# MIC-DKFZ/MultiTalent

Hardware: AMD Instinct MI355X
Metric: CT patches/s (48x192x192) train fwd+bwd (higher is better)
Workload: dtype f32; 1 GPU; Task009_Spleen Generic_UNet nc=2 softmax Dice+CE; batch_per_gpu=2, global_batch=2, parallelism=dp1, step=fwd+loss+bwd+clip12+SGD-nesterov, precision=fp32

## Files before the change

### include/mtseg.h

```cpp
#ifndef MTSEG_H
#define MTSEG_H

#include <stddef.h>
#include <stdint.h>

#ifdef __cplusplus
extern "C" {
#endif

#define MT_OK 0
#define MT_EINVAL (-1)
#define MT_EWORKSPACE (-2)
#define MT_EHIP (-3)
#define MT_EUNSUPPORTED (-4)

#define MT_ABI_VERSION 4
#define MT_MAX_CHUNKS 64

#define MT_F32 0
#define MT_BF16 1
#define MT_F16 2

typedef void* mt_stream_t;

// ... 104 lines not shown
  float* stats_part;
  int32_t odtype;
  int32_t scatter;
  int32_t mma;
} mt_pointwise_t;
int mt_pointwise_fwd(const mt_pointwise_t* p, mt_stream_t stream);
int mt_pointwise_stats_blocks(const mt_pointwise_t* p);
int mt_pointwise_io_supported(const mt_pointwise_t* p);
int mt_pointwise_pack_layout(const mt_pointwise_t* p);
int mt_head_bwd_supported(int Cin, int Cout);
size_t mt_head_bwd_workspace(int N, long V, int Cin, int Cout);
int mt_head_bwd(const mt_src_t* x, const float* dy, int dycs, int N, long V, int Cin, int Cout, const float* wpack_bwd,
                float* dx, int dxcs, int dxdtype , int accumulate_dx, float* dw,
                long s_ci, long s_co, float* dbias, int accumulate_dw, int* dbias_done, void* ws, size_t ws_bytes, mt_stream_t stream);
int mt_head_bwd_io_supported(int xdtype, int xcs, int dxdtype, int dxcs, int Cin, int Cout);


int mt_inorm_finalize(const float* part, int N, int nsb, int C, double count, const float* gamma,
                      const float* beta, float eps, float* mean, float* rstd, float* scale, float* shift,
                      mt_stream_t stream);
int mt_inorm_lrelu_apply(const float* y, int ycs, const float* scale, const float* shift, float slope,
                         const float* res, int rcs, const float* rscale, const float* rshift, float rslope,
                         float* out, int ocs, int N, long V, int C, int dtype , mt_stream_t stream);
size_t mt_inorm_bwd_workspace(int N, long V, int C);
int mt_inorm_lrelu_bwd(float* g, int gcs, const float* y, int ycs, const float* mean, const float* rstd,
                       const float* gamma, const float* beta, float slope, int N, long V, int C,
                       float* dgamma, float* dbeta, float* dbias, const float* part, int part_nblk, int part_cs, int part_c0,
                       void* ws, size_t ws_bytes, int gdtype, int ydtype , mt_stream_t stream);
int mt_lrelu_bwd(float* g, int gcs, const float* y, int ycs, const float* scale, const float* shift,
                 float slope, const float* y2, int y2cs, const float* scale2, const float* shift2,
// ... 131 lines not shown
```

### multitalent_amd/_lib.py

```python
import ctypes as C
import os

_HERE = os.path.dirname(os.path.abspath(__file__))
LIB_PATH = os.path.join(_HERE, os.environ.get('MT_LIB_VARIANT', 'libmtseg_hip.so'))

MT_MAX_CHUNKS = 64
c_float_p = C.POINTER(C.c_float)


class mt_src_t(C.Structure):
    _fields_ = [('ptr', C.c_void_p), ('cs', C.c_int32), ('C', C.c_int32), ('scale', C.c_void_p),
                ('shift', C.c_void_p), ('slope', C.c_float), ('dtype', C.c_int32)]


class mt_bwd_stats_t(C.Structure):
    _fields_ = [('y', C.c_void_p), ('mean', C.c_void_p), ('rstd', C.c_void_p), ('gamma', C.c_void_p), ('beta', C.c_void_p),
                ('ycs', C.c_int32), ('c0', C.c_int32), ('C', C.c_int32), ('slope', C.c_float)]


class mt_conv3d_t(C.Structure):
    _fields_ = [('src', mt_src_t * 2), ('nsrc', C.c_int32),
                ('N', C.c_int32), ('Di', C.c_int32), ('Hi', C.c_int32), ('Wi', C.c_int32),
                ('dilD', C.c_int32), ('dilH', C.c_int32), ('dilW', C.c_int32),
                ('Do', C.c_int32), ('Ho', C.c_int32), ('Wo', C.c_int32),
# ... 53 lines not shown
    'mt_gaussian_blur_axis': (_i, [_vp, _vp, _i, _i, _i, _i, _i, _vp, _vp]),
    'mt_conv3d_pack_layout': (_i, [_P(mt_conv3d_t)]),
    'mt_conv3d_bwd_data_strided_pack_layout': (_i, [_P(mt_conv3d_t)]),
    'mt_conv3d_kernel_name': (_i, [_P(mt_conv3d_t), C.c_char_p, _sz]),
    'mt_conv3d_bwd_stats_supported': (_i, [_P(mt_conv3d_t)]),
    'mt_conv3d_bwd_weight_kernel_name': (_i, [_P(mt_conv3d_t), _P(mt_src_t), C.c_char_p, _sz]),
    'mt_conv3d_bwd_data_strided_kernel_name': (_i, [_P(mt_conv3d_t), C.c_char_p, _sz]),
    'mt_conv3d_bwd_weight_workspace': (_sz, [_P(mt_conv3d_t)]),
    'mt_conv3d_bwd_weight': (_i, [_P(mt_conv3d_t), _P(mt_src_t), _vp, _l, _l, _l, _l, _l, _i, _vp, _sz, _vp]),
    'mt_pointwise_fwd': (_i, [_P(mt_pointwise_t), _vp]),
    'mt_pointwise_stats_blocks': (_i, [_P(mt_pointwise_t)]),
    'mt_head_bwd_supported': (_i, [_i, _i]),
    'mt_head_bwd_workspace': (_sz, [_i, _l, _i, _i]),
    'mt_head_bwd': (_i, [_P(mt_src_t), _vp, _i, _i, _l, _i, _i, _vp, _vp, _i, _i, _i, _vp, _l, _l, _vp, _i, _P(C.c_int), _vp, _sz, _vp]),
    'mt_head_bwd_io_supported': (_i, [_i, _i, _i, _i, _i, _i]),
    'mt_pointwise_io_supported': (_i, [_P(mt_pointwise_t)]),
    'mt_pointwise_pack_layout': (_i, [_P(mt_pointwise_t)]),
    'mt_inorm_finalize': (_i, [_vp, _i, _i, _i, _d, _vp, _vp, _f, _vp, _vp, _vp, _vp, _vp]),
    'mt_inorm_lrelu_apply': (_i, [_vp, _i, _vp, _vp, _f, _vp, _i, _vp, _vp, _f, _vp, _i, _i, _l, _i, _i, _vp]),
    'mt_inorm_bwd_workspace': (_sz, [_i, _l, _i]),
    'mt_inorm_lrelu_bwd': (_i, [_vp, _i, _vp, _i, _vp, _vp, _vp, _vp, _f, _i, _l, _i, _vp, _vp, _vp, _vp, _i, _i, _i, _vp, _sz, _i, _i, _vp]),
    'mt_lrelu_bwd': (_i, [_vp, _i, _vp, _i, _vp, _vp, _f, _vp, _i, _vp, _vp, _f, _vp, _i, _i, _l, _i, _i, _i, _vp]),
    'mt_lrelu_bwd_stats_blocks': (_i, [_l, _i]),
    'mt_lrelu_bwd_stats': (_i, [_vp, _vp, _vp, _vp, _f, _vp, _vp, _vp, _f, _vp, _vp, _vp, _vp, _i, _l, _i, _i, _i, _vp]),
    'mt_channel_sum_workspace': (_sz, [_i, _l, _i]),
    'mt_channel_sum': (_i, [_vp, _i, _i, _l, _i, _vp, _i, _vp, _sz, _i, _vp]),
    'mt_cast': (_i, [_vp, _i, _i, _vp, _i, _i, _l, _i, _i, _vp]),
    'mt_conv3d_io_supported': (_i, [_P(mt_conv3d_t)]),
    'mt_conv3d_bwd_data_strided_io_supported': (_i, [_P(mt_conv3d_t)]),
    'mt_conv3d_bwd_weight_io_supported': (_i, [_P(mt_conv3d_t), _P(mt_src_t)]),
# ... 105 lines not shown
```

### multitalent_amd/csrc/mt_common.h

```cpp
#pragma once
#include <hip/hip_runtime.h>
#include <stdint.h>
#include <stdio.h>
#include "../../include/mtseg.h"

typedef __attribute__((ext_vector_type(16))) float f32x16;
typedef __attribute__((ext_vector_type(4))) float f32x4;

#define MT_WAVE 64

void mt_set_error(const char* fmt, ...);

#define MT_REQUIRE(cond, ...)            \
  do {                                   \
    if (!(cond)) {                       \
      mt_set_error(__VA_ARGS__);         \
      return MT_EINVAL;                  \
    }                                    \
  } while (0)

#define MT_REQUIRE_WORKSPACE(who, have, need)                                              \
  do {                                                                                   \
    const size_t have_ = (have), need_ = (need);                                         \
    if (have_ < need_) {                                                                 \
      mt_set_error("%s: workspace of %zu bytes, %zu needed", who, have_, need_);         \
      return MT_EWORKSPACE;                                                              \
// ... 130 lines not shown
```

### multitalent_amd/csrc/norm.hip

```cpp
#include "mt_common.h"
#include <initializer_list>

__global__ __launch_bounds__(256) void inorm_finalize_kernel(const float* __restrict__ part, int nsb, int C, double count,
                                                             const float* __restrict__ gamma, const float* __restrict__ beta,
                                                             float eps, float* mean, float* rstd, float* scale, float* shift) {
  __shared__ double red[4][2];
  const int n = blockIdx.x / C, c = blockIdx.x % C;
  const float2* p = (const float2*)part + (size_t)n * nsb * C + c;
  double s1 = 0.0, s2 = 0.0;
  for (int s = threadIdx.x; s < nsb; s += 256) {
    const float2 v = p[(size_t)s * C];
    s1 += (double)v.x; s2 += (double)v.y;
  }
  s1 = mt_wave_sum_d(s1);
  s2 = mt_wave_sum_d(s2);
  if ((threadIdx.x & 63) == 0) { red[threadIdx.x >> 6][0] = s1; red[threadIdx.x >> 6][1] = s2; }
  __syncthreads();
  if (threadIdx.x == 0) {
    s1 = (red[0][0] + red[1][0]) + (red[2][0] + red[3][0]);
    s2 = (red[0][1] + red[1][1]) + (red[2][1] + red[3][1]);
    const double m = s1 / count;
    double var = s2 / count - m * m;
    if (var < 0.0) var = 0.0;
    const double rs = 1.0 / sqrt(var + (double)eps);
// ... 212 lines not shown
  a = mt_wave_sum_d(a);
  if (threadIdx.x == 0) out[c] = accumulate ? out[c] + (float)a : (float)a;
}


#define NF_UNROLL 4

struct InBwdFast {
  void* g; const void* y;
  const float* mean; const float* rstd; const float* gamma; const float* beta; float slope;
  long nvec;
  int C, G, A, nblk;
  float* part1;
  const float* m;
  float* part2;
};

template <int VEC, bool APPLY, int AT, int GT>
__global__ __launch_bounds__(256) void inorm_bwd_fast_kernel(const InBwdFast P) {
  static_assert(mt_ebytes<AT>() == mt_ebytes<GT>(), "one vector index addresses both tensors");
  __shared__ float red[256 * VEC * 2];
  const int n = blockIdx.y, t = threadIdx.x;
  const bool act = t < P.A;
  const int grp = t % P.G;
  float mu[VEC], rs[VEC], ga[VEC], be[VEC], m1[VEC], m2[VEC], a0[VEC], a1[VEC];
#pragma unroll
  for (int e = 0; e < VEC; ++e) {
    const int c = grp * VEC + e;
    mu[e] = P.mean[(size_t)n * P.C + c]; rs[e] = P.rstd[(size_t)n * P.C + c];
    ga[e] = P.gamma ? P.gamma[c] : 1.f; be[e] = P.beta ? P.beta[c] : 0.f;
    if (APPLY) { m1[e] = P.m[((size_t)n * P.C + c) * 2]; m2[e] = P.m[((size_t)n * P.C + c) * 2 + 1]; }
    a0[e] = 0.f; a1[e] = 0.f;
  }
  const long per = ((P.nvec + P.nblk - 1) / P.nblk + P.A - 1) / P.A * P.A;
  const long lo = (long)blockIdx.x * per;
  long hi = lo + per; if (hi > P.nvec) hi = P.nvec;
  const size_t sbytes = (size_t)n * P.nvec * VEC * mt_ebytes<GT>();
  char* gp = (char*)P.g + sbytes;
  const char* yp = (const char*)P.y + sbytes;
  if (act) {
    for (long i0 = lo + t; i0 < hi; i0 += (long)P.A * NF_UNROLL) {
      float gv[NF_UNROLL][VEC], yv[NF_UNROLL][VEC];
#pragma unroll
      for (int u = 0; u < NF_UNROLL; ++u) {
        const long i = i0 + (long)u * P.A;
        if (i < hi) { mt_ldv<VEC, GT>(gp, (size_t)i, gv[u]); mt_ldv<VEC, AT>(yp, (size_t)i, yv[u]); }
      }
#pragma unroll
      for (int u = 0; u < NF_UNROLL; ++u) {
        const long i = i0 + (long)u * P.A;
        if (i < hi) {
          float out[VEC];
#pragma unroll
          for (int e = 0; e < VEC; ++e) {
            const float zh = (yv[u][e] - mu[e]) * rs[e];
            const float z = fmaf(zh, ga[e], be[e]);
            float dz = gv[u][e];
            dz = z > 0.f ? dz : dz * P.slope;
            if (APPLY) {
              const float dy = mt_round_st<GT>(ga[e] * rs[e] * (dz - m1[e] - zh * m2[e]));
              out[e] = dy;
              a0[e] += dy;
            } else {
              a0[e] += dz;
              a1[e] = fmaf(dz, zh, a1[e]);
            }
          }
          if (APPLY) mt_stv<VEC, GT>(gp, (size_t)i, out);
        }
      }
    }
// ... 123 lines not shown
static void inorm_bwd_fast_dispatch(const InBwdFast& F, dim3 grid, int vec, int at, int gt, bool reduce, hipStream_t st) {
  if (at == MT_F32) {
    if (vec == 4) launch_inorm_bwd_fast<4, MT_F32, MT_F32>(F, grid, reduce, st);
    else if (vec == 2) launch_inorm_bwd_fast<2, MT_F32, MT_F32>(F, grid, reduce, st);
    else launch_inorm_bwd_fast<1, MT_F32, MT_F32>(F, grid, reduce, st);
  } else if (at == MT_F16) {
    if (vec == 8) launch_inorm_bwd_fast<8, MT_F16, MT_BF16>(F, grid, reduce, st);
    else if (vec == 4) launch_inorm_bwd_fast<4, MT_F16, MT_BF16>(F, grid, reduce, st);
    else launch_inorm_bwd_fast<2, MT_F16, MT_BF16>(F, grid, reduce, st);
  } else {
    if (vec == 8) launch_inorm_bwd_fast<8, MT_BF16, MT_BF16>(F, grid, reduce, st);
    else if (vec == 4) launch_inorm_bwd_fast<4, MT_BF16, MT_BF16>(F, grid, reduce, st);
    else launch_inorm_bwd_fast<2, MT_BF16, MT_BF16>(F, grid, reduce, st);
  }
}
extern "C" int mt_inorm_lrelu_bwd(float* g, int gcs, const float* y, int ycs, const float* mean, const float* rstd,
                                  const float* gamma, const float* beta, float slope, int N, long V, int C,
                                  float* dgamma, float* dbeta, float* dbias, const float* part, int part_nblk, int part_cs, int part_c0,
                                  void* ws, size_t ws_bytes, int gdtype, int ydtype, mt_stream_t stream) {
  MT_REQUIRE(g && y && mean && rstd && N > 0 && V > 0 && C > 0 && mt_dtype_ok(gdtype) && mt_dtype_ok(ydtype), "inorm_lrelu_bwd: bad args");
  MT_REQUIRE(part == nullptr || (part_nblk > 0 && part_cs >= part_c0 + C && part_c0 >= 0), "inorm_lrelu_bwd: bad external partials");
  if (ws == nullptr || ws_bytes < mt_inorm_bwd_workspace(N, V, C)) { mt_set_error("inorm_lrelu_bwd: workspace too small"); return MT_EWORKSPACE; }
  InBwdParams P;
  P.g = g; P.gcs = gcs; P.y = y; P.ycs = ycs; P.mean = mean; P.rstd = rstd; P.gamma = gamma; P.beta = beta; P.slope = slope;
  P.V = V; P.C = C; P.nvb = nb_blocks(V);
  float* w = (float*)ws;
  P.part1 = w; w += (size_t)N * P.nvb * C * 2;
  P.m = w; w += (size_t)N * C * 2;
  P.part2 = dbias ? w : nullptr;
  P.p1 = part ? part : P.part1; P.p1_nblk = part ? part_nblk : P.nvb; P.p1_cs = part ? part_cs : C; P.p1_c0 = part ? part_c0 : 0;
  P.gt = gdtype; P.at = ydtype;
  hipStream_t st = (hipStream_t)stream;
  const int vec = (gcs == C && ycs == C && ag_fast(ydtype, gdtype)) ? dense_vec(C, V * C, gdtype, {g, y}) : 0;
  const bool contig = vec > 0 && (C / vec <= 256);
  constexpr int small_on = 1;
  const int svec = gdtype == MT_F32 ? 4 : 8;
  if (small_on && contig && part == nullptr && vec == svec && (long)N * V <= INORM_SMALL_MAX) {
    InBwdSmall S;
    S.g = g; S.y = y; S.mean = mean; S.rstd = rstd; S.gamma = gamma; S.beta = beta; S.slope = slope; S.V = V; S.C = C; S.N = N;
    S.dgamma = dgamma; S.dbeta = dbeta; S.dbias = dbias;
    const dim3 grid(C / svec);
    const dim3 blk(V > 768 ? 1024 : V > 512 ? 768 : V > 256 ? 512 : 256);
    if (gdtype == MT_F32) hipLaunchKernelGGL((inorm_bwd_small_kernel<4, MT_F32, MT_F32>), grid, blk, 0, st, S);
    else if (ydtype == MT_F16) hipLaunchKernelGGL((inorm_bwd_small_kernel<8, MT_F16, MT_BF16>), grid, blk, 0, st, S);
    else hipLaunchKernelGGL((inorm_bwd_small_kernel<8, MT_BF16, MT_BF16>), grid, blk, 0, st, S);
    MT_CHECK_LAUNCH("inorm_lrelu_bwd(small)");
    return MT_OK;
  }
  if (contig) {
    InBwdFast F;
    F.g = g; F.y = y; F.mean = mean; F.rstd = rstd; F.gamma = gamma; F.beta = beta; F.slope = slope;
    F.nvec = (long)V * C / vec; F.C = C; F.G = C / vec; F.A = (256 / F.G) * F.G; F.nblk = P.nvb;
    F.part1 = P.part1; F.m = P.m; F.part2 = P.part2;
    dim3 grid(P.nvb, N);
    if (part == nullptr) inorm_bwd_fast_dispatch(F, grid, vec, ydtype, gdtype, true, st);
    hipLaunchKernelGGL(inorm_bwd_finalize_kernel, dim3(C), dim3(256), 0, st, P, N, dgamma, dbeta);
    inorm_bwd_fast_dispatch(F, grid, vec, ydtype, gdtype, false, st);
  } else {
    if (part == nullptr) hipLaunchKernelGGL(inorm_bwd_reduce_kernel, dim3(P.nvb, N), dim3(256), 0, st, P);
    hipLaunchKernelGGL(inorm_bwd_finalize_kernel, dim3(C), dim3(256), 0, st, P, N, dgamma, dbeta);
    hipLaunchKernelGGL(inorm_bwd_apply_kernel, dim3(P.nvb, N), dim3(256), 0, st, P);
  }
  if (dbias) hipLaunchKernelGGL(colsum_kernel, dim3(C), dim3(64), 0, st, (const float*)P.part2, (long)N * P.nvb, C, dbias, 0);
  MT_CHECK_LAUNCH("inorm_lrelu_bwd");
  return MT_OK;
}

struct LBwdParams {
  void* g; int gcs; const void* y; int ycs; const float* scale; const float* shift; float slope;
  const void* y2; int y2cs; const float* scale2; const float* shift2; float slope2;
  void* gcopy; int gcopycs; long V; int C;
  int gt, at;
};
__global__ __launch_bounds__(256) void lrelu_bwd_kernel(const LBwdParams P) {
  const int n = blockIdx.y;
  const int cl = threadIdx.x & 31, vr = threadIdx.x >> 5;
  const int vb = mt_vb(P.V);
  const long v0 = (long)blockIdx.x * vb;
  const long v1 = (v0 + vb < P.V) ? v0 + vb : P.V;
  for (int cb = 0; cb < P.C; cb += 32) {
// ... 392 lines not shown
```

### multitalent_amd/csrc/pointwise.hip

```cpp
#include "mt_common.h"
#include <stdlib.h>
#include <string.h>

struct PwKParams {
  mt_pointwise_t c;
  int ntaps, nchunks, nsb;
  long Vb;
  int wide;
};

#define PW_MAXC 1024
#define PW_CK 16

__device__ __forceinline__ void pw_pair_exchange(float vj, float vj1, bool odd, float& a, float& b) {
  const float send = odd ? vj : vj1;
  const float recv = __builtin_bit_cast(float, __builtin_amdgcn_mov_dpp(__builtin_bit_cast(int, send), 0xB1 , 0xF, 0xF, true));
  a = odd ? recv : vj;
  b = odd ? vj1 : recv;
}
__device__ __forceinline__ float pw_pair_combine(float s0, float s1, bool odd) {
  const float t0 = __builtin_bit_cast(float, __builtin_amdgcn_mov_dpp(__builtin_bit_cast(int, s0), 0xB1, 0xF, 0xF, true));
  const float t1 = __builtin_bit_cast(float, __builtin_amdgcn_mov_dpp(__builtin_bit_cast(int, s1), 0xB1, 0xF, 0xF, true));
  return odd ? s1 + t1 : s0 + t0;
}
// ... 973 lines not shown
      else PW_LAUNCH(8);
      break;
    }
  }
#undef PW_LAUNCH
#undef PW_LAUNCH_T
  MT_CHECK_LAUNCH("pointwise");
  return MT_OK;
}


struct HeadBwdParams {
  mt_src_t x; const float* dy; int dycs; int N; long V; int Cin, Cout;
  const float* wpack; float* dx; int dxcs; int accumulate_dx;
  float* part; int nwaves; long ntiles;
};
template <int NCI, int XS = MT_F32, int OS = MT_F32, bool ST = false>
__global__ __launch_bounds__(256) void head_bwd_kernel(const HeadBwdParams P) {
  constexpr int XE = mt_ebytes<XS>(), OE = mt_ebytes<OS>();
  constexpr int HB_WF = 2048 + 1024 * NCI;
  __shared__ __attribute__((aligned(16))) float hb_img[ST ? 4 * HB_WF : 4];
  static_assert(!ST || 4 * HB_WF * sizeof(float) <= 65536, "head_bwd_kernel: the four wave images must fit the 64 KiB of static LDS (NCI <= 2)");
  const int tid = threadIdx.x, lane = tid & 63;
  const int wave = __builtin_amdgcn_readfirstlane(tid >> 6);
  float* const idy = hb_img + (ST ? wave * HB_WF : 0);
  float* const ixf = idy + (ST ? 2048 : 0);
  const int li = lane & 31, lhalf = lane >> 5;
  const int gw = blockIdx.x * 4 + wave;
  const mt_src_t& S = P.x;
  const bool aff = S.scale != nullptr;
// ... 257 lines not shown
  } else {
#pragma unroll
    for (int q = 0; q < CIN / 2; ++q) { const unsigned d = *(const unsigned*)(row + q * 4); x[2 * q] = mt_lo16<ST>(d); x[2 * q + 1] = mt_hi16<ST>(d); }
  }
}
template <int CIN, int ST>
__device__ __forceinline__ void hn_row_to_lds(char* row, const float (&x)[CIN + 2]) {
  if constexpr (ST == MT_F32) {
#pragma unroll
    for (int q = 0; q < CIN / 2; ++q) { float2 t; t.x = x[2 * q]; t.y = x[2 * q + 1]; *(float2*)(row + q * 8) = t; }
  } else {
#pragma unroll
    for (int q = 0; q < CIN / 2; ++q) *(unsigned*)(row + q * 4) = mt_pk16<ST>(x[2 * q], x[2 * q + 1]);
  }
}
template <int CIN, int NCO, int XS = MT_F32, int OS = MT_F32>
__global__ __launch_bounds__(256) void head_bwd_narrow_kernel(const HeadBwdParams P) {
  static_assert(CIN % 2 == 0, "channel pairs");
  __shared__ __attribute__((aligned(16))) float hn_img[4 * 64 * CIN];
  constexpr int XE = mt_ebytes<XS>(), OE = mt_ebytes<OS>();
  constexpr int NP = NCO * CIN + NCO;
  __shared__ __attribute__((aligned(16))) float sw[NCO][CIN + 2], ssc[CIN + 2], ssh[CIN + 2];
  __shared__ float red[4][NP];
  const int tid = threadIdx.x, lane = tid & 63;
  const int wave = __builtin_amdgcn_readfirstlane(tid >> 6);
  const mt_src_t& S = P.x;
  const bool aff = S.scale != nullptr;
  const float slope = aff ? S.slope : 1.f;
  for (int i = tid; i < NCO * CIN; i += 256) {
    const int co = i / CIN, ci = i - co * CIN;
    sw[co][ci] = co < P.Cout ? P.wpack[ci * 4 + co] : 0.f;
  }
  float part[NP];
#pragma unroll
  for (int k = 0; k < NP; ++k) part[k] = 0.f;
  const long per_sample_blocks = HN_BLOCKS / P.N > 0 ? HN_BLOCKS / P.N : 1;
  const int nb = (int)(blockIdx.x / per_sample_blocks);
  if (nb < P.N) {
    const long b = blockIdx.x - (long)nb * per_sample_blocks;
    for (int i = tid; i < CIN; i += 256) {
      ssc[i] = aff ? S.scale[(size_t)nb * S.C + i] : 1.f;
      ssh[i] = aff ? S.shift[(size_t)nb * S.C + i] : 0.f;
    }
    __syncthreads();
    const size_t xs = (size_t)P.V * CIN;
    __amdgpu_buffer_rsrc_t ra = __builtin_amdgcn_make_buffer_rsrc((void*)((const char*)S.ptr + (size_t)nb * xs * XE), 0, (int)(xs * XE), 0x00020000);
    __amdgpu_buffer_rsrc_t rx = __builtin_amdgcn_make_buffer_rsrc((void*)((char*)P.dx + (size_t)nb * xs * OE), 0, (int)(xs * OE), 0x00020000);
    const float* dyp = P.dy + (size_t)nb * P.V * P.dycs;
    constexpr int ROWX = CIN * XE, ROWO = CIN * OE;
    constexpr int NPX = 64 * ROWX / 16, NPO = 64 * ROWO / 16;
    char* const img = (char*)hn_img + wave * (64 * CIN * 4);
    for (long v0 = b * 256 + wave * 64; v0 < P.V; v0 += per_sample_blocks * 256) {
      const long v = v0 + lane;
      const bool vok = v < P.V;
      float x[CIN + 2], old[CIN + 2], dy[NCO];
      {
        uint4 pc[(NPX + 63) / 64];
// ... 33 lines not shown
      }
#pragma unroll
      for (int co = 0; co < NCO; ++co) dy[co] = (vok && co < P.Cout) ? dyp[v * P.dycs + co] : 0.f;
      float dx[CIN + 2];
#pragma unroll
      for (int ci = 0; ci < CIN; ++ci) {
        const float t = fmaf(x[ci], ssc[ci], ssh[ci]);
        const float a = fmaxf(t, t * slope);
        float g = P.accumulate_dx ? old[ci] : 0.f;
#pragma unroll
        for (int co = 0; co < NCO; ++co) {
          g = fmaf(dy[co], sw[co][ci], g);
          part[co * CIN + ci] = fmaf(a, dy[co], part[co * CIN + ci]);
        }
        dx[ci] = g;
      }
#pragma unroll
      for (int co = 0; co < NCO; ++co) part[NCO * CIN + co] += dy[co];
      hn_row_to_lds<CIN, OS>(img + lane * ROWO, dx);
      __builtin_amdgcn_s_waitcnt(0xc07f);
      __builtin_amdgcn_wave_barrier();
#pragma unroll
      for (int k = 0; k < (NPO + 63) / 64; ++k) {
        const int p = k * 64 + lane;
        if (p < NPO) {
          const uint4 q = *(const uint4*)(img + p * 16);
          __builtin_amdgcn_raw_buffer_store_b128(__builtin_bit_cast(__attribute__((ext_vector_type(4))) unsigned, q), rx, (int)(v0 * ROWO) + p * 16, 0, 0);
        }
      }
      __builtin_amdgcn_s_waitcnt(0xc07f);
      __builtin_amdgcn_wave_barrier();
    }
  }
#pragma unroll
  for (int k = 0; k < NP; ++k) {
    float s = part[k];
#pragma unroll
    for (int off = 32; off > 0; off >>= 1) s += __shfl_xor(s, off, 64);
    if (lane == 0) red[wave][k] = s;
  }
  __syncthreads();
  for (int k = tid; k < NP; k += 256) P.part[(size_t)blockIdx.x * NP + k] = (red[0][k] + red[1][k]) + (red[2][k] + red[3][k]);
}
__global__ __launch_bounds__(64) void head_narrow_reduce_kernel(const float* part, int nblocks, int np, int Cin, int Cout, int nco, float* dw, long s_ci,
                                                               long s_co, float* dbias, int accumulate) {
  const int k = blockIdx.x;
  double s = 0.0;
  for (int b = threadIdx.x; b < nblocks; b += 64) s += (double)part[(size_t)b * np + k];
  s = mt_wave_sum_d(s);
  if (threadIdx.x != 0) return;
  const int co = k < nco * Cin ? k / Cin : k - nco * Cin, ci = k < nco * Cin ? k - co * Cin : -1;
  if (co >= Cout) return;
  if (ci >= 0) { float* o = dw + (long)ci * s_ci + (long)co * s_co; *o = accumulate ? *o + (float)s : (float)s; }
  else if (dbias != nullptr) dbias[co] = accumulate ? dbias[co] + (float)s : (float)s;
}
static bool head_bwd_narrow_ok(const mt_src_t* x, int dycs, int dxcs, int Cin, int Cout, long V, int N, const float* dx) {
  constexpr int use = 1;
// ... 68 lines not shown
  else { if (nci == 1) HB(1, false); else HB(2, false); }
#undef HB
  MT_CHECK_LAUNCH("head_bwd");
  HeadBwdReduce R;
  R.part = (const float*)ws; R.nwaves = P.nwaves; R.nci = nci; R.Cin = Cin; R.Cout = Cout; R.dw = dw; R.s_ci = s_ci; R.s_co = s_co;
  R.dbias = dbias; R.accumulate = accumulate_dw;
  const size_t per = (size_t)nci * 2 * 1024;
  R.tmp = (double*)(((uintptr_t)((float*)ws + (size_t)P.nwaves * per) + 7) & ~(uintptr_t)7);
  hipLaunchKernelGGL(head_bwd_reduce_a_kernel, dim3(mt_cdiv((long)per, 256), HB_SLICES), dim3(256), 0, st, R);
  hipLaunchKernelGGL(head_bwd_reduce_b_kernel, dim3(mt_cdiv((long)per, 256)), dim3(256), 0, st, R);
  MT_CHECK_LAUNCH("head_bwd_reduce");
  if (dbias_done != nullptr) *dbias_done = ((Cin % 32) != 0) ? 1 : 0;
  return MT_OK;
}


__global__ void probe_straddle_kernel(const float* p, int nrec_bytes, float* out) {
  __amdgpu_buffer_rsrc_t r = __builtin_amdgcn_make_buffer_rsrc((void*)p, 0, nrec_bytes, 0x00020000);
  const int off = threadIdx.x * 8;
  f32x4 v = __builtin_bit_cast(f32x4, __builtin_amdgcn_raw_buffer_load_b128(r, off, 0, 0));
  for (int e = 0; e < 4; ++e) out[threadIdx.x * 4 + e] = v[e];
}
__global__ void probe_unaligned_kernel(const float* p, int nrec_bytes, float* out) {
  __amdgpu_buffer_rsrc_t r = __builtin_amdgcn_make_buffer_rsrc((void*)p, 0, nrec_bytes, 0x00020000);
  const int off = (threadIdx.x * 47 + 1) * 4;
  f32x4 v = __builtin_bit_cast(f32x4, __builtin_amdgcn_raw_buffer_load_b128(r, off, 0, 0));
  for (int e = 0; e < 4; ++e) out[threadIdx.x * 4 + e] = v[e];
}

extern "C" int mt_probe_device(void* scratch, size_t scratch_bytes, int* vector_loads_ok, char* arch, size_t arch_len, mt_stream_t stream) {
// ... 38 lines not shown
```

### multitalent_amd/engine.py

```python
import contextlib
import os

import torch
from torch import nn

from . import ops
from .ops import Act, ConvGeom

LRELU_DEFAULT = 1e-2


class Val:

    def __init__(self, name, C):
        self.name, self.C = name, C
        self.act = None
        self.grad = None
        self.grad_init = False
        self.spatial = None


class _Op:
    params = ()

# ... 12 lines not shown


class ConvNormOp(_Op):

    def __init__(self, name, srcs, out, conv, norm, lrelu=True, pointwise=False):
        self.name, self.srcs, self.out, self.conv, self.norm, self.lrelu = name, srcs, out, conv, norm, lrelu
        self.kernel = tuple(conv.kernel_size)
        self.stride = tuple(conv.stride)
        self.pad = tuple(conv.padding)
        self.slope = LRELU_DEFAULT
        self.pointwise = pointwise
        self._pw_strided_geom = (not pointwise and self.kernel == (1, 1, 1) and self.stride != (1, 1, 1) and self.pad == (0, 0, 0)
                                 and len(srcs) == 1)
        self.pw_strided = False
        self.bwd_part = None

    def inputs(self):
        return list(self.srcs)

    def param_list(self):
        ps = [self.conv.weight]
        if self.conv.bias is not None:
            ps.append(self.conv.bias)
        if self.norm is not None:
            ps += [self.norm.weight, self.norm.bias]
        return ps

    def plan(self, eng, N):
        dev = eng.device
        sp = self.srcs[0].spatial
# ... 134 lines not shown
        geomT = ConvGeom(self.geom.out, self.kernel, (1, 1, 1), tuple(k - 1 - p for k, p in zip(self.kernel, self.pad)),
                         dil=self.stride, out_spatial=self.geom.inp)
        gact = Act(g) if g is not None else Act(self._grad_like(eng, self.out))
        outs = [Act(self._grad_like(eng, s)) for s in self.srcs]

        def build(ins, outs_):
            return ops.fill_conv(ins, geomT, Cin, out0=outs_[0], out1=outs_[1] if len(outs_) > 1 else None,
                                 csplit=self.srcs[0].C if len(outs_) > 1 else None, mma=self.mma)
        return eng.io(self.name + '.bwdd', [gact], outs, build, ops.conv_io_supported, grad_ins=True)

    def backward(self, eng):
        g = self.out.grad
        assert g is not None and self.out.grad_init, "gradient of %s was never produced" % self.name
        gact = Act(g)
        dbias = eng.grad_of(self.conv.bias) if self.conv.bias is not None else None
        if self.norm is not None:
            a = self.out.act
            ws = eng.workspace(ops.inorm_bwd_workspace(a.N, a.V, a.C))
            part, part_c0 = self.bwd_part if self.bwd_part is not None else (None, 0)
            self.bwd_part = None
            ops.inorm_lrelu_bwd(gact, a, self.norm.weight, self.norm.bias, eng.grad_of(self.norm.weight),
                                eng.grad_of(self.norm.bias), dbias, ws, part=part, part_c0=part_c0)
        elif dbias is not None:
            ws = eng.workspace(ops.channel_sum_workspace(gact.N, gact.V, gact.C))
            ops.channel_sum(gact, dbias, False, ws)
        dw = eng.grad_of(self.conv.weight)
        with eng.weight_stream() as side:
            iow = eng.io(self.name + '.bwdw', [s.act for s in self.srcs] + [gact], [],
                         lambda ins, outs: (ops.fill_conv(ins[:-1], self.geom, self.conv.out_channels, mma=self.mma), ins[-1]),
                         lambda py: ops.conv_bwd_weight_io_supported(py[0], py[1]), grad_ins=[False] * len(self.srcs) + [True])
            pw, yact = iow.build()
# ... 238 lines not shown

    def _out_dtype(self, eng):
        return torch.float32

    def backward(self, eng):
        s0 = self.srcs[0]
        Cout = self.conv.out_channels
        if s0.grad is None or self.wb is None or not ops.head_bwd_supported(s0.C, Cout) or self.stride != (1, 1, 1):
            return super().backward(eng)
        g = self.out.grad
        assert g is not None and self.out.grad_init, "gradient of %s was never produced" % self.name
        gact = Act(g)
        dbias = eng.grad_of(self.conv.bias) if self.conv.bias is not None else None
        w = self.conv.weight
        st = _strides(w)
        io = eng.io(self.name + '.hbwd', [s0.act], [Act(s0.grad)], lambda ins, outs: (ins[0], outs[0]),
                    lambda xo: ops.head_bwd_io_supported(xo[0], xo[1], Cout))
        a, dx = io.build()
        io.pre()
        ws = eng.workspace(ops.head_bwd_workspace(a.N, a.V, s0.C, Cout))
        done = ops.head_bwd(a, gact, self.wb, dx, bool(io.accumulate(s0.grad_init)), eng.grad_of(w), st[0], st[1], dbias, False, ws)
        io.post(s0.grad_init)
        if dbias is not None and not done:
            ws2 = eng.workspace(ops.channel_sum_workspace(gact.N, gact.V, gact.C))
            ops.channel_sum(gact, dbias, False, ws2)
        s0.grad_init = True


class _IO:

    def __init__(self, eng, key, ins, outs, build, flags, grad_ins):
        self.eng, self._build = eng, build
        cast_in, cast_out = flags
        self.native = not (cast_in or cast_out)
        self._cin = [(a, g) for a, g in zip(ins, grad_ins) if cast_in and a.dtype != torch.float32]
        self.ins = [eng.as_fp32(a, geometry_only=True) if (cast_in and a.dtype != torch.float32) else a for a in ins]
        self._cout = []
        self.outs = []
        for i, o in enumerate(outs):
            if cast_out and o.dtype != torch.float32:
                t = Act(eng.buffer('%s.out%d' % (key, i), tuple(o.buf.shape[:4]) + (o.C,)))
# ... 37 lines not shown
        self.params_version = 0
        self.wstreams = []
        self._wnext = 0
        self._late_pack = None
        self._mid_pack = None
        self._ws_side = {}
        self.bwdw_streams = int(os.environ.get('MT_BWDW_STREAMS', '1'))
        self.grad_ready_hook = None
        self.dummy = None
        self.mma = 0
        self._io_cache = {}
        self._fp32_copies = {}
        self._iter = 0
        self.io_cast_bytes = 0
        self._fuse_norm_bwd = None
        self._one_stream_at_init = self.bwdw_streams == 0
        self.producer, self.pending = {}, {}

    @property
    def fuse_norm_bwd(self):
        if self._fuse_norm_bwd is not None:
            return int(self._fuse_norm_bwd)
        if self._one_stream_at_init:
            return 1
        return 3 if self.mma else 0

    @fuse_norm_bwd.setter
    def fuse_norm_bwd(self, v):
        self._fuse_norm_bwd = v

# ... 452 lines not shown
```

### multitalent_amd/ops.py

```python
import ctypes as C
import os

import numpy as np
import torch

from . import _lib
from ._lib import mt_conv3d_t, mt_pointwise_t, mt_src_t


def _stream():
    return C.c_void_p(torch.cuda.current_stream().cuda_stream)


def _ptr(t):
    return C.c_void_p(t.data_ptr()) if t is not None else C.c_void_p(0)


def _check_dev(*ts):
    for t in ts:
        if t is not None and not t.is_cuda:
            raise RuntimeError("multitalent_amd ops require HIP device tensors (no CPU fallback)")


_DT_CODES = {torch.float32: _lib.MT_F32, torch.bfloat16: _lib.MT_BF16, torch.float16: _lib.MT_F16}
# ... 367 lines not shown
    assert dy.dt == _lib.MT_F32, "mt_head_bwd reads the fp32 loss gradient"
    xs = x.src()
    done = C.c_int(0)
    _lib.check(lib.mt_head_bwd(C.byref(xs), C.c_void_p(dy.data_ptr()), dy.cs, x.N, x.V, x.C, dy.C, _ptr(wpack_bwd),
                               C.c_void_p(dx.data_ptr()), dx.cs, dx.dt, int(accumulate_dx), _ptr(dw), int(s_ci), int(s_co), _ptr(dbias),
                               int(accumulate_dw), C.byref(done), _ptr(ws), ws.numel() * ws.element_size(), _stream()), 'head_bwd')
    return bool(done.value)


def head_bwd_io_supported(x, dx, Cout):
    return bool(_lib.load().mt_head_bwd_io_supported(x.dt, x.cs, dx.dt, dx.cs, x.C, int(Cout)))


def head_bwd_workspace(N, V, Cin, Cout):
    return _lib.load().mt_head_bwd_workspace(int(N), int(V), int(Cin), int(Cout))


def pointwise_stats_blocks(p):
    return _lib.load().mt_pointwise_stats_blocks(C.byref(p))


def inorm_finalize(part, N, nsb, Cn, count, gamma, beta, eps, mean, rstd, scale, shift):
    _lib.check(_lib.load().mt_inorm_finalize(_ptr(part), N, nsb, Cn, float(count), _ptr(gamma), _ptr(beta), float(eps),
                                             _ptr(mean), _ptr(rstd), _ptr(scale), _ptr(shift), _stream()), 'inorm_finalize')


def inorm_lrelu_apply(y, out, res=None):
    _lib.check(_lib.load().mt_inorm_lrelu_apply(
        C.c_void_p(y.data_ptr()), y.cs, _ptr(y.scale), _ptr(y.shift), y.slope,
        C.c_void_p(res.data_ptr()) if res is not None else None, res.cs if res is not None else 0,
# ... 663 lines not shown
```

Baseline: 67.45 patches/s.

## Fuse segmentation head backward with preceding instance-norm/LeakyReLU backward

Adds a fused path where the 1x1x1 head backward kernel also computes the instance-norm backward first-pass statistics (sum of dz and dz*zhat) from the head's input gradient. It skips writing that gradient to memory. The norm apply pass then recomputes the input gradient on the fly from dy and the head weights instead of reading a materialised gradient tensor. This saves a full-resolution write plus reread at the highest-resolution level, at the cost of extra compute and more template variants. The path is enabled by default when the producer is a conv+norm+lrelu op with fp32 dense tensors.

```diff
diff --git a/include/mtseg.h b/include/mtseg.h
--- a/include/mtseg.h
+++ b/include/mtseg.h
@@ -142,6 +142,13 @@
                 float* dx, int dxcs, int dxdtype , int accumulate_dx, float* dw,
                 long s_ci, long s_co, float* dbias, int accumulate_dw, int* dbias_done, void* ws, size_t ws_bytes, mt_stream_t stream);
 int mt_head_bwd_io_supported(int xdtype, int xcs, int dxdtype, int dxcs, int Cin, int Cout);
+int mt_head_norm_bwd_supported(const mt_src_t* y, const float* dy, int dycs, int N, long V, int Cin, int Cout, const float* draw,
+                               int drawcs, int drawdtype, int accumulate_dx);
+size_t mt_head_norm_bwd_workspace(int N, long V, int Cin, int Cout);
+int mt_head_norm_bwd(const mt_src_t* y, const float* mean, const float* rstd, const float* gamma, const float* beta,
+                     const float* dy, int dycs, int N, long V, int Cin, int Cout, const float* wpack_bwd,
+                     float* draw, float* dw, long s_ci, long s_co, float* dbias_head,
+                     float* dgamma, float* dbeta, float* dbias_conv, void* ws, size_t ws_bytes, mt_stream_t stream);
 
 
 int mt_inorm_finalize(const float* part, int N, int nsb, int C, double count, const float* gamma,
diff --git a/multitalent_amd/_lib.py b/multitalent_amd/_lib.py
--- a/multitalent_amd/_lib.py
+++ b/multitalent_amd/_lib.py
@@ -91,6 +91,9 @@
     'mt_head_bwd_workspace': (_sz, [_i, _l, _i, _i]),
     'mt_head_bwd': (_i, [_P(mt_src_t), _vp, _i, _i, _l, _i, _i, _vp, _vp, _i, _i, _i, _vp, _l, _l, _vp, _i, _P(C.c_int), _vp, _sz, _vp]),
     'mt_head_bwd_io_supported': (_i, [_i, _i, _i, _i, _i, _i]),
+    'mt_head_norm_bwd_supported': (_i, [_P(mt_src_t), _vp, _i, _i, _l, _i, _i, _vp, _i, _i, _i]),
+    'mt_head_norm_bwd_workspace': (_sz, [_i, _l, _i, _i]),
+    'mt_head_norm_bwd': (_i, [_P(mt_src_t), _vp, _vp, _vp, _vp, _vp, _i, _i, _l, _i, _i, _vp, _vp, _vp, _l, _l, _vp, _vp, _vp, _vp, _vp, _sz, _vp]),
     'mt_pointwise_io_supported': (_i, [_P(mt_pointwise_t)]),
     'mt_pointwise_pack_layout': (_i, [_P(mt_pointwise_t)]),
     'mt_inorm_finalize': (_i, [_vp, _i, _i, _i, _d, _vp, _vp, _f, _vp, _vp, _vp, _vp, _vp]),
diff --git a/multitalent_amd/csrc/mt_common.h b/multitalent_amd/csrc/mt_common.h
--- a/multitalent_amd/csrc/mt_common.h
+++ b/multitalent_amd/csrc/mt_common.h
@@ -10,6 +10,10 @@
 #define MT_WAVE 64
 
 void mt_set_error(const char* fmt, ...);
+
+int mt_inorm_bwd_from_head(float* draw, const float* y, const float* mean, const float* rstd, const float* gamma, const float* beta, float slope,
+                           int N, long V, int C, float* dgamma, float* dbeta, float* dbias, const float* part1, int p1_nblk,
+                           const float* dy, int dycs, int hcout, const float* hwpack, void* ws, size_t ws_bytes, hipStream_t st);
 
 #define MT_REQUIRE(cond, ...)            \
   do {                                   \
diff --git a/multitalent_amd/csrc/norm.hip b/multitalent_amd/csrc/norm.hip
--- a/multitalent_amd/csrc/norm.hip
+++ b/multitalent_amd/csrc/norm.hip
@@ -250,11 +250,14 @@
   float* part1;
   const float* m;
   float* part2;
+  const float* hdy; int hdycs, hcout; const float* hw;
 };
 
-template <int VEC, bool APPLY, int AT, int GT>
+template <int VEC, bool APPLY, int AT, int GT, int HCO = 0>
 __global__ __launch_bounds__(256) void inorm_bwd_fast_kernel(const InBwdFast P) {
   static_assert(mt_ebytes<AT>() == mt_ebytes<GT>(), "one vector index addresses both tensors");
+  static_assert(HCO == 0 || (APPLY && GT == MT_F32), "the head form is the fp32 apply pass");
+  constexpr int NH = HCO > 0 ? HCO : 1;
   __shared__ float red[256 * VEC * 2];
   const int n = blockIdx.y, t = threadIdx.x;
   const bool act = t < P.A;
@@ -268,20 +271,36 @@
     if (APPLY) { m1[e] = P.m[((size_t)n * P.C + c) * 2]; m2[e] = P.m[((size_t)n * P.C + c) * 2 + 1]; }
     a0[e] = 0.f; a1[e] = 0.f;
   }
+  float hw[NH][VEC];
+  if constexpr (HCO > 0) {
+#pragma unroll
+    for (int co = 0; co < HCO; ++co)
+#pragma unroll
+      for (int e = 0; e < VEC; ++e) hw[co][e] = co < P.hcout ? P.hw[(grp * VEC + e) * 4 + co] : 0.f;
+  }
   const long per = ((P.nvec + P.nblk - 1) / P.nblk + P.A - 1) / P.A * P.A;
   const long lo = (long)blockIdx.x * per;
   long hi = lo + per; if (hi > P.nvec) hi = P.nvec;
   const size_t sbytes = (size_t)n * P.nvec * VEC * mt_ebytes<GT>();
   char* gp = (char*)P.g + sbytes;
   const char* yp = (const char*)P.y + sbytes;
+  const long vstep = P.A / P.G;
+  const float* hdy = HCO > 0 ? P.hdy + ((size_t)n * (size_t)(P.nvec / P.G) + (size_t)((lo + t) / P.G)) * P.hdycs : nullptr;
   if (act) {
     for (long i0 = lo + t; i0 < hi; i0 += (long)P.A * NF_UNROLL) {
-      float gv[NF_UNROLL][VEC], yv[NF_UNROLL][VEC];
+      float gv[NF_UNROLL][VEC], yv[NF_UNROLL][VEC], dl[NF_UNROLL][NH];
 #pragma unroll
       for (int u = 0; u < NF_UNROLL; ++u) {
         const long i = i0 + (long)u * P.A;
-        if (i < hi) { mt_ldv<VEC, GT>(gp, (size_t)i, gv[u]); mt_ldv<VEC, AT>(yp, (size_t)i, yv[u]); }
-      }
+        if (i < hi) {
+          if constexpr (HCO > 0) {
+#pragma unroll
+            for (int co = 0; co < HCO; ++co) dl[u][co] = co < P.hcout ? hdy[(size_t)(u * vstep) * P.hdycs + co] : 0.f;
+          } else mt_ldv<VEC, GT>(gp, (size_t)i, gv[u]);
+          mt_ldv<VEC, AT>(yp, (size_t)i, yv[u]);
+        }
+      }
+      if constexpr (HCO > 0) hdy += (size_t)(NF_UNROLL * vstep) * P.hdycs;
 #pragma unroll
       for (int u = 0; u < NF_UNROLL; ++u) {
         const long i = i0 + (long)u * P.A;
@@ -291,6 +310,12 @@
           for (int e = 0; e < VEC; ++e) {
             const float zh = (yv[u][e] - mu[e]) * rs[e];
             const float z = fmaf(zh, ga[e], be[e]);
+            if constexpr (HCO > 0) {
+              float g = 0.f;
+#pragma unroll
+              for (int co = 0; co < HCO; ++co) g = fmaf(dl[u][co], hw[co][e], g);
+              gv[u][e] = g;
+            }
             float dz = gv[u][e];
             dz = z > 0.f ? dz : dz * P.slope;
             if (APPLY) {
@@ -444,10 +469,11 @@
     else launch_inorm_bwd_fast<2, MT_BF16, MT_BF16>(F, grid, reduce, st);
   }
 }
-extern "C" int mt_inorm_lrelu_bwd(float* g, int gcs, const float* y, int ycs, const float* mean, const float* rstd,
-                                  const float* gamma, const float* beta, float slope, int N, long V, int C,
-                                  float* dgamma, float* dbeta, float* dbias, const float* part, int part_nblk, int part_cs, int part_c0,
-                                  void* ws, size_t ws_bytes, int gdtype, int ydtype, mt_stream_t stream) {
+struct InHeadGrad { const float* dy; int dycs, cout; const float* wpack; };
+static int inorm_lrelu_bwd_impl(float* g, int gcs, const float* y, int ycs, const float* mean, const float* rstd,
+                                const float* gamma, const float* beta, float slope, int N, long V, int C,
+                                float* dgamma, float* dbeta, float* dbias, const float* part, int part_nblk, int part_cs, int part_c0,
+                                void* ws, size_t ws_bytes, int gdtype, int ydtype, const InHeadGrad* hg, mt_stream_t stream) {
   MT_REQUIRE(g && y && mean && rstd && N > 0 && V > 0 && C > 0 && mt_dtype_ok(gdtype) && mt_dtype_ok(ydtype), "inorm_lrelu_bwd: bad args");
   MT_REQUIRE(part == nullptr || (part_nblk > 0 && part_cs >= part_c0 + C && part_c0 >= 0), "inorm_lrelu_bwd: bad external partials");
   if (ws == nullptr || ws_bytes < mt_inorm_bwd_workspace(N, V, C)) { mt_set_error("inorm_lrelu_bwd: workspace too small"); return MT_EWORKSPACE; }
@@ -465,6 +491,8 @@
   const bool contig = vec > 0 && (C / vec <= 256);
   constexpr int small_on = 1;
   const int svec = gdtype == MT_F32 ? 4 : 8;
+  MT_REQUIRE(hg == nullptr || (contig && part != nullptr && gdtype == MT_F32 && vec == (C % 4 ? 2 : 4) && hg->cout >= 1 && hg->cout <= 4),
+             "inorm_lrelu_bwd: the head-gradient form takes dense, 16-byte aligned fp32 tensors with first-pass partials");
   if (small_on && contig && part == nullptr && vec == svec && (long)N * V <= INORM_SMALL_MAX) {
     InBwdSmall S;
     S.g = g; S.y = y; S.mean = mean; S.rstd = rstd; S.gamma = gamma; S.beta = beta; S.slope = slope; S.V = V; S.C = C; S.N = N;
@@ -482,10 +510,15 @@
     F.g = g; F.y = y; F.mean = mean; F.rstd = rstd; F.gamma = gamma; F.beta = beta; F.slope = slope;
     F.nvec = (long)V * C / vec; F.C = C; F.G = C / vec; F.A = (256 / F.G) * F.G; F.nblk = P.nvb;
     F.part1 = P.part1; F.m = P.m; F.part2 = P.part2;
+    F.hdy = hg ? hg->dy : nullptr; F.hdycs = hg ? hg->dycs : 0; F.hcout = hg ? hg->cout : 0; F.hw = hg ? hg->wpack : nullptr;
     dim3 grid(P.nvb, N);
     if (part == nullptr) inorm_bwd_fast_dispatch(F, grid, vec, ydtype, gdtype, true, st);
     hipLaunchKernelGGL(inorm_bwd_finalize_kernel, dim3(C), dim3(256), 0, st, P, N, dgamma, dbeta);
-    inorm_bwd_fast_dispatch(F, grid, vec, ydtype, gdtype, false, st);
+    if (hg == nullptr) inorm_bwd_fast_dispatch(F, grid, vec, ydtype, gdtype, false, st);
+    else if (vec == 2 && hg->cout <= 2) hipLaunchKernelGGL((inorm_bwd_fast_kernel<2, true, MT_F32, MT_F32, 2>), grid, dim3(256), 0, st, F);
+    else if (vec == 2) hipLaunchKernelGGL((inorm_bwd_fast_kernel<2, true, MT_F32, MT_F32, 4>), grid, dim3(256), 0, st, F);
+    else if (hg->cout <= 2) hipLaunchKernelGGL((inorm_bwd_fast_kernel<4, true, MT_F32, MT_F32, 2>), grid, dim3(256), 0, st, F);
+    else hipLaunchKernelGGL((inorm_bwd_fast_kernel<4, true, MT_F32, MT_F32, 4>), grid, dim3(256), 0, st, F);
   } else {
     if (part == nullptr) hipLaunchKernelGGL(inorm_bwd_reduce_kernel, dim3(P.nvb, N), dim3(256), 0, st, P);
     hipLaunchKernelGGL(inorm_bwd_finalize_kernel, dim3(C), dim3(256), 0, st, P, N, dgamma, dbeta);
@@ -494,6 +527,20 @@
   if (dbias) hipLaunchKernelGGL(colsum_kernel, dim3(C), dim3(64), 0, st, (const float*)P.part2, (long)N * P.nvb, C, dbias, 0);
   MT_CHECK_LAUNCH("inorm_lrelu_bwd");
   return MT_OK;
+}
+extern "C" int mt_inorm_lrelu_bwd(float* g, int gcs, const float* y, int ycs, const float* mean, const float* rstd,
+                                  const float* gamma, const float* beta, float slope, int N, long V, int C,
+                                  float* dgamma, float* dbeta, float* dbias, const float* part, int part_nblk, int part_cs, int part_c0,
+                                  void* ws, size_t ws_bytes, int gdtype, int ydtype, mt_stream_t stream) {
+  return inorm_lrelu_bwd_impl(g, gcs, y, ycs, mean, rstd, gamma, beta, slope, N, V, C, dgamma, dbeta, dbias, part, part_nblk, part_cs, part_c0,
+                              ws, ws_bytes, gdtype, ydtype, nullptr, stream);
+}
+int mt_inorm_bwd_from_head(float* draw, const float* y, const float* mean, const float* rstd, const float* gamma, const float* beta, float slope,
+                           int N, long V, int C, float* dgamma, float* dbeta, float* dbias, const float* part1, int p1_nblk,
+                           const float* dy, int dycs, int hcout, const float* hwpack, void* ws, size_t ws_bytes, hipStream_t st) {
+  const InHeadGrad hg = {dy, dycs, hcout, hwpack};
+  return inorm_lrelu_bwd_impl(draw, C, y, C, mean, rstd, gamma, beta, slope, N, V, C, dgamma, dbeta, dbias, part1, p1_nblk, C, 0,
+                              ws, ws_bytes, MT_F32, MT_F32, &hg, (mt_stream_t)st);
 }
 
 struct LBwdParams {
diff --git a/multitalent_amd/csrc/pointwise.hip b/multitalent_amd/csrc/pointwise.hip
--- a/multitalent_amd/csrc/pointwise.hip
+++ b/multitalent_amd/csrc/pointwise.hip
@@ -1011,6 +1011,7 @@
   mt_src_t x; const float* dy; int dycs; int N; long V; int Cin, Cout;
   const float* wpack; float* dx; int dxcs; int accumulate_dx;
   float* part; int nwaves; long ntiles;
+  const float* nmean; const float* nrstd; const float* ngamma; const float* nbeta; float* npart;
 };
 template <int NCI, int XS = MT_F32, int OS = MT_F32, bool ST = false>
 __global__ __launch_bounds__(256) void head_bwd_kernel(const HeadBwdParams P) {
@@ -1298,9 +1299,16 @@
     for (int q = 0; q < CIN / 2; ++q) *(unsigned*)(row + q * 4) = mt_pk16<ST>(x[2 * q], x[2 * q + 1]);
   }
 }
-template <int CIN, int NCO, int XS = MT_F32, int OS = MT_F32>
+template <int CIN, int NCO, int XS = MT_F32, int OS = MT_F32, bool NB = false>
 __global__ __launch_bounds__(256) void head_bwd_narrow_kernel(const HeadBwdParams P) {
   static_assert(CIN % 2 == 0, "channel pairs");
+  static_assert(!NB || (XS == MT_F32 && OS == MT_F32), "the norm-backward form is fp32 only");
+  constexpr int NS = NB ? CIN : 1;
+  __shared__ float smu[NS + 2], srs[NS + 2], sga[NS + 2], sbe[NS + 2];
+  __shared__ float red2[4][2 * NS];
+  float st0[NS], st1[NS];
+#pragma unroll
+  for (int k = 0; k < NS; ++k) { st0[k] = 0.f; st1[k] = 0.f; }
   __shared__ __attribute__((aligned(16))) float hn_img[4 * 64 * CIN];
   constexpr int XE = mt_ebytes<XS>(), OE = mt_ebytes<OS>();
   constexpr int NP = NCO * CIN + NCO;
@@ -1325,6 +1333,10 @@
     for (int i = tid; i < CIN; i += 256) {
       ssc[i] = aff ? S.scale[(size_t)nb * S.C + i] : 1.f;
       ssh[i] = aff ? S.shift[(size_t)nb * S.C + i] : 0.f;
+      if constexpr (NB) {
+        smu[i] = P.nmean[(size_t)nb * CIN + i]; srs[i] = P.nrstd[(size_t)nb * CIN + i];
+        sga[i] = P.ngamma ? P.ngamma[i] : 1.f; sbe[i] = P.nbeta ? P.nbeta[i] : 0.f;
+      }
     }
     __syncthreads();
     const size_t xs = (size_t)P.V * CIN;
@@ -1388,9 +1400,17 @@
           part[co * CIN + ci] = fmaf(a, dy[co], part[co * CIN + ci]);
         }
         dx[ci] = g;
+        if constexpr (NB) {
+          const float zh = (x[ci] - smu[ci]) * srs[ci];
+          const float z = fmaf(zh, sga[ci], sbe[ci]);
+          const float dz = z > 0.f ? g : g * S.slope;
+          st0[ci] += dz;
+          st1[ci] = fmaf(dz, zh, st1[ci]);
+        }
       }
 #pragma unroll
       for (int co = 0; co < NCO; ++co) part[NCO * CIN + co] += dy[co];
+      if constexpr (NB) continue;
       hn_row_to_lds<CIN, OS>(img + lane * ROWO, dx);
       __builtin_amdgcn_s_waitcnt(0xc07f);
       __builtin_amdgcn_wave_barrier();
@@ -1415,6 +1435,18 @@
   }
   __syncthreads();
   for (int k = tid; k < NP; k += 256) P.part[(size_t)blockIdx.x * NP + k] = (red[0][k] + red[1][k]) + (red[2][k] + red[3][k]);
+  if constexpr (NB) {
+#pragma unroll
+    for (int c = 0; c < CIN; ++c) {
+      float s0 = st0[c], s1 = st1[c];
+#pragma unroll
+      for (int off = 32; off > 0; off >>= 1) { s0 += __shfl_xor(s0, off, 64); s1 += __shfl_xor(s1, off, 64); }
+      if (lane == 0) { red2[wave][2 * c] = s0; red2[wave][2 * c + 1] = s1; }
+    }
+    __syncthreads();
+    if (nb < P.N)
+      for (int k = tid; k < 2 * CIN; k += 256) P.npart[(size_t)blockIdx.x * 2 * CIN + k] = (red2[0][k] + red2[1][k]) + (red2[2][k] + red2[3][k]);
+  }
 }
 __global__ __launch_bounds__(64) void head_narrow_reduce_kernel(const float* part, int nblocks, int np, int Cin, int Cout, int nco, float* dw, long s_ci,
                                                                long s_co, float* dbias, int accumulate) {
@@ -1513,6 +1545,53 @@
   return MT_OK;
 }
 
+static inline int hnb_per_sample(int N) { return HN_BLOCKS / N > 0 ? HN_BLOCKS / N : 1; }
+static inline size_t hnb_align(size_t b) { return (b + 255) & ~(size_t)255; }
+extern "C" int mt_head_norm_bwd_supported(const mt_src_t* y, const float* dy, int dycs, int N, long V, int Cin, int Cout, const float* draw,
+                                          int drawcs, int drawdtype, int accumulate_dx) {
+  if (y == nullptr || y->ptr == nullptr || dy == nullptr || draw == nullptr || N <= 0 || V <= 0) return 0;
+  if (y->dtype != MT_F32 || drawdtype != MT_F32 || accumulate_dx) return 0;
+  if (!(Cin == 30 || Cin == 32) || Cout < 1 || Cout > 4 || y->C != Cin) return 0;
+  if (y->scale == nullptr || y->shift == nullptr || !(y->slope >= 0.f && y->slope <= 1.f)) return 0;
+  if (!head_bwd_narrow_ok(y, dycs, drawcs, Cin, Cout, V, N, draw)) return 0;
+  if ((((uintptr_t)y->ptr) | ((uintptr_t)draw)) & 15) return 0;
+  if (dycs < Cout || (double)V * dycs * 4.0 >= 2147483648.0) return 0;
+  return 1;
+}
+extern "C" size_t mt_head_norm_bwd_workspace(int N, long V, int Cin, int Cout) {
+  if (!(N > 0 && V > 0 && (Cin == 30 || Cin == 32) && Cout >= 1 && Cout <= 4)) return 0;
+  const int nco = Cout <= 2 ? 2 : 4, np = nco * Cin + nco, nblocks = hnb_per_sample(N) * N;
+  return hnb_align((size_t)nblocks * np * sizeof(float)) + hnb_align((size_t)nblocks * Cin * 2 * sizeof(float)) + mt_inorm_bwd_workspace(N, V, Cin);
+}
+extern "C" int mt_head_norm_bwd(const mt_src_t* y, const float* mean, const float* rstd, const float* gamma, const float* beta,
+                                const float* dy, int dycs, int N, long V, int Cin, int Cout, const float* wpack_bwd,
+                                float* draw, float* dw, long s_ci, long s_co, float* dbias_head,
+                                float* dgamma, float* dbeta, float* dbias_conv, void* ws, size_t ws_bytes, mt_stream_t stream) {
+  MT_REQUIRE(y && mean && rstd && wpack_bwd && dw, "head_norm_bwd: null argument");
+  MT_REQUIRE(mt_head_norm_bwd_supported(y, dy, dycs, N, V, Cin, Cout, draw, Cin, MT_F32, 0), "head_norm_bwd: case not taken (ask mt_head_norm_bwd_supported)");
+  MT_REQUIRE_WORKSPACE("head_norm_bwd", ws ? ws_bytes : 0, mt_head_norm_bwd_workspace(N, V, Cin, Cout));
+  const int nco = Cout <= 2 ? 2 : 4, np = nco * Cin + nco;
+  const int per_sample = hnb_per_sample(N), nblocks = per_sample * N;
+  char* w = (char*)ws;
+  HeadBwdParams P;
+  P.x = *y; P.dy = dy; P.dycs = dycs; P.N = N; P.V = V; P.Cin = Cin; P.Cout = Cout; P.wpack = wpack_bwd;
+  P.dx = draw; P.dxcs = Cin; P.accumulate_dx = 0; P.nwaves = 0; P.ntiles = 0;
+  P.part = (float*)w; w += hnb_align((size_t)nblocks * np * sizeof(float));
+  P.npart = (float*)w; w += hnb_align((size_t)nblocks * Cin * 2 * sizeof(float));
+  P.nmean = mean; P.nrstd = rstd; P.ngamma = gamma; P.nbeta = beta;
+  hipStream_t st = (hipStream_t)stream;
+#define HBN(CIN_, NCO_) hipLaunchKernelGGL((head_bwd_narrow_kernel<CIN_, NCO_, MT_F32, MT_F32, true>), dim3(nblocks), dim3(256), 0, st, P)
+  if (Cin == 30 && nco == 2) HBN(30, 2);
+  else if (Cin == 30) HBN(30, 4);
+  else if (nco == 2) HBN(32, 2);
+  else HBN(32, 4);
+#undef HBN
+  hipLaunchKernelGGL(head_narrow_reduce_kernel, dim3(np), dim3(64), 0, st, (const float*)P.part, nblocks, np, Cin, Cout, nco, dw, s_ci, s_co, dbias_head, 0);
+  MT_CHECK_LAUNCH("head_norm_bwd");
+  return mt_inorm_bwd_from_head(draw, (const float*)y->ptr, mean, rstd, gamma, beta, y->slope, N, V, Cin, dgamma, dbeta, dbias_conv,
+                                P.npart, per_sample, dy, dycs, Cout, wpack_bwd, w, ws_bytes - (size_t)(w - (char*)ws), st);
+}
+
 
 __global__ void probe_straddle_kernel(const float* p, int nrec_bytes, float* out) {
   __amdgpu_buffer_rsrc_t r = __builtin_amdgcn_make_buffer_rsrc((void*)p, 0, nrec_bytes, 0x00020000);
diff --git a/multitalent_amd/engine.py b/multitalent_amd/engine.py
--- a/multitalent_amd/engine.py
+++ b/multitalent_amd/engine.py
@@ -50,6 +50,7 @@
                                  and len(srcs) == 1)
         self.pw_strided = False
         self.bwd_part = None
+        self.norm_bwd_done = False
 
     def inputs(self):
         return list(self.srcs)
@@ -214,7 +215,9 @@
         assert g is not None and self.out.grad_init, "gradient of %s was never produced" % self.name
         gact = Act(g)
         dbias = eng.grad_of(self.conv.bias) if self.conv.bias is not None else None
-        if self.norm is not None:
+        if self.norm is not None and self.norm_bwd_done:
+            self.norm_bwd_done = False
+        elif self.norm is not None:
             a = self.out.act
             ws = eng.workspace(ops.inorm_bwd_workspace(a.N, a.V, a.C))
             part, part_c0 = self.bwd_part if self.bwd_part is not None else (None, 0)
@@ -483,6 +486,8 @@
         dbias = eng.grad_of(self.conv.bias) if self.conv.bias is not None else None
         w = self.conv.weight
         st = _strides(w)
+        if self._head_norm_bwd(eng, gact, dbias, w, st):
+            return
         io = eng.io(self.name + '.hbwd', [s0.act], [Act(s0.grad)], lambda ins, outs: (ins[0], outs[0]),
                     lambda xo: ops.head_bwd_io_supported(xo[0], xo[1], Cout))
         a, dx = io.build()
@@ -494,6 +499,28 @@
             ws2 = eng.workspace(ops.channel_sum_workspace(gact.N, gact.V, gact.C))
             ops.channel_sum(gact, dbias, False, ws2)
         s0.grad_init = True
+
+
+    def _head_norm_bwd(self, eng, gact, dbias, w, st):
+        s0 = self.srcs[0]
+        if not (eng.fuse_bwd_ends & 1) or s0.grad_init or eng.pending.get(id(s0), 0) != 1:
+            return False
+        prod = eng.producer.get(id(s0))
+        if (not isinstance(prod, ConvNormOp) or isinstance(prod, HeadOp) or prod.norm is None or not prod.lrelu or prod.bwd_part is not None
+                or s0.act.buf is not prod.out.act.buf):
+            return False
+        a, draw = s0.act, Act(s0.grad)
+        if not ops.head_norm_bwd_supported(a, gact, draw, False):
+            return False
+        Cout = self.conv.out_channels
+        ws = eng.workspace(ops.head_norm_bwd_workspace(a.N, a.V, a.C, Cout))
+        ops.head_norm_bwd(a, gact, self.wb, prod.norm.weight, prod.norm.bias, draw, eng.grad_of(w), st[0], st[1], dbias,
+                          eng.grad_of(prod.norm.weight), eng.grad_of(prod.norm.bias),
+                          eng.grad_of(prod.conv.bias) if prod.conv.bias is not None else None, ws)
+        prod.norm_bwd_done = True
+        s0.grad_init = True
+        eng.bwd_ends_launches[0] += 1
+        return True
 
 
 class _IO:
@@ -561,6 +588,8 @@
         self._iter = 0
         self.io_cast_bytes = 0
         self._fuse_norm_bwd = None
+        self.fuse_bwd_ends = 1
+        self.bwd_ends_launches = [0, 0]
         self._one_stream_at_init = self.bwdw_streams == 0
         self.producer, self.pending = {}, {}
 
diff --git a/multitalent_amd/ops.py b/multitalent_amd/ops.py
--- a/multitalent_amd/ops.py
+++ b/multitalent_amd/ops.py
@@ -405,6 +405,27 @@
 
 def head_bwd_workspace(N, V, Cin, Cout):
     return _lib.load().mt_head_bwd_workspace(int(N), int(V), int(Cin), int(Cout))
+
+
+def head_norm_bwd_supported(y, dy, draw, accumulate_dx):
+    if y.scale is None or y.mean is None or y.rstd is None:
+        return False
+    ys = y.src()
+    return bool(_lib.load().mt_head_norm_bwd_supported(C.byref(ys), C.c_void_p(dy.data_ptr()), dy.cs, y.N, y.V, y.C, dy.C,
+                                                       C.c_void_p(draw.data_ptr()), draw.cs, draw.dt, int(bool(accumulate_dx))))
+
+
+def head_norm_bwd_workspace(N, V, Cin, Cout):
+    return _lib.load().mt_head_norm_bwd_workspace(int(N), int(V), int(Cin), int(Cout))
+
+
+def head_norm_bwd(y, dy, wpack_bwd, gamma, beta, draw, dw, s_ci, s_co, dbias_head, dgamma, dbeta, dbias_conv, ws):
+    assert dy.dt == _lib.MT_F32 and draw.dt == _lib.MT_F32 and draw.cs == y.C
+    ys = y.src()
+    _lib.check(_lib.load().mt_head_norm_bwd(
+        C.byref(ys), _ptr(y.mean), _ptr(y.rstd), _ptr(gamma), _ptr(beta), C.c_void_p(dy.data_ptr()), dy.cs, y.N, y.V, y.C, dy.C,
+        _ptr(wpack_bwd), C.c_void_p(draw.data_ptr()), _ptr(dw), int(s_ci), int(s_co), _ptr(dbias_head), _ptr(dgamma), _ptr(dbeta),
+        _ptr(dbias_conv), _ptr(ws), ws.numel() * ws.element_size(), _stream()), 'head_norm_bwd')
 
 
 def pointwise_stats_blocks(p):
```

Result: no change. 67.94 patches/s, median of 6 (+0.7%).
